# CILAB-MA/gpudrive_lab

Hardware: AMD Instinct MI355X
Metric: agent-steps/sec at 1024 worlds x 64 agents; achieved HBM GB/s on obs kernel (higher is better)
Workload: dtype f32

## Files before the change

### gpudrive_lab_amd/csrc/map_obs_rank.hip

```cpp
#include <hip/hip_runtime.h>

#include <algorithm>
#include <type_traits>

#include "engine.hpp"
#include "gd_math.hpp"
#include "rank_heap.hpp"

namespace gd {

namespace {

constexpr int K = GD_MAP_OBS_K;
constexpr int CAP = GD_RANK_CAP;
constexpr int NCP = GD_RANK_NCP;
constexpr int SPL = GD_RANK_SPL;
constexpr int KT = GD_RANK_KT;
constexpr int TILE = 32;
constexpr int CAP_LONG = GD_RANK_CAP_LONG;
template <int CAP_T>
struct RankGeo {
    static constexpr bool LONG = CAP_T > CAP;
    static constexpr int NG = CAP_T / 64;
    static constexpr int NMAX = CAP_T - 8;
    static constexpr int NB = CAP_T;
    static constexpr int NLIN = CAP_T * 3 / 5;
    static constexpr int TSH = LONG ? 6 : 5;
    static constexpr int RSH = LONG ? 4 : 5;
    static constexpr int KTN = LONG ? GD_RANK_KT_LONG : GD_RANK_KT;
};
constexpr int NB = RankGeo<CAP>::NB;
static_assert(K + (NCP - 1) * TILE >= CAP && K + (NCP - 1) * 64 >= CAP_LONG, "a checkpoint slot for every tile of candidates");
static_assert(CAP % 64 == 0 && NB % 128 == 0 && CAP < 2047 && CAP_LONG % 640 == 0 && CAP_LONG < 4095, "geometry; less + 1 fits 11 / 12 bits");
static_assert(SPL >= K + 31 && SPL <= CAP && KT >= CAP / 16 + 1, "every slot the finish looks up; an entry per 16 slots + the last");
constexpr int RK_FAR = 1 << 30;
constexpr int RK_TIES = 1 << 30;

__device__ __forceinline__ void wave_sync() {
    __builtin_amdgcn_fence(__ATOMIC_RELEASE, "wavefront");
    __builtin_amdgcn_wave_barrier();
    __builtin_amdgcn_fence(__ATOMIC_ACQUIRE, "wavefront");
}

__device__ __forceinline__ int wave_incl_scan(int v) {
    v += __builtin_amdgcn_update_dpp(0, v, 0x111, 0xf, 0xf, false);
    v += __builtin_amdgcn_update_dpp(0, v, 0x112, 0xf, 0xf, false);
    v += __builtin_amdgcn_update_dpp(0, v, 0x114, 0xf, 0xf, false);
    v += __builtin_amdgcn_update_dpp(0, v, 0x118, 0xf, 0xf, false);
    v += __builtin_amdgcn_update_dpp(0, v, 0x142, 0xa, 0xf, false);
    v += __builtin_amdgcn_update_dpp(0, v, 0x143, 0xc, 0xf, false);
    return v;
}

#define GD_DPP_SELF(v, ctrl, rows) __builtin_amdgcn_update_dpp((v), (v), (ctrl), (rows), 0xf, false)
__device__ __forceinline__ int wave_max(int v) {
    v = max(v, GD_DPP_SELF(v, 0x111, 0xf));
    v = max(v, GD_DPP_SELF(v, 0x112, 0xf));
    v = max(v, GD_DPP_SELF(v, 0x114, 0xf));
    v = max(v, GD_DPP_SELF(v, 0x118, 0xf));
    v = max(v, GD_DPP_SELF(v, 0x142, 0xa));
    v = max(v, GD_DPP_SELF(v, 0x143, 0xc));
    return __builtin_amdgcn_readlane(v, 63);
}
__device__ __forceinline__ float wave_max_nonneg(float f) { return __int_as_float(wave_max(__float_as_int(f))); }
__device__ __forceinline__ float wave_min_nonneg(float f) { return __int_as_float(~wave_max(~__float_as_int(f))); }
__device__ __forceinline__ int wave_sum(int v) { return __builtin_amdgcn_readlane(wave_incl_scan(v), 63); }

#ifndef GD_NT_SCAN_STORE
#define GD_NT_SCAN_STORE 0
#endif
#ifndef GD_NT_WORDS_LOAD
#define GD_NT_WORDS_LOAD 1
#endif
#ifndef GD_NT_FINISH_LOAD
#define GD_NT_FINISH_LOAD 1
#endif
#ifndef GD_NT_REPLAY_LOAD
#define GD_NT_REPLAY_LOAD 1
#endif
typedef unsigned int u4v __attribute__((ext_vector_type(4)));
typedef unsigned int u2v __attribute__((ext_vector_type(2)));
template <typename T>
__device__ __forceinline__ T stream_load(const T *p) { return __builtin_nontemporal_load(p); }
template <typename T>
__device__ __forceinline__ void stream_store(T v, T *p) { __builtin_nontemporal_store(v, p); }
__device__ __forceinline__ uint4 stream_load(const uint4 *p) {
    const u4v v = __builtin_nontemporal_load(reinterpret_cast<const u4v *>(p));
    return make_uint4(v.x, v.y, v.z, v.w);
}
__device__ __forceinline__ void stream_store(uint4 v, uint4 *p) {
    u4v t; t.x = v.x; t.y = v.y; t.z = v.z; t.w = v.w;
    __builtin_nontemporal_store(t, reinterpret_cast<u4v *>(p));
}
__device__ __forceinline__ uint2 stream_load(const uint2 *p) {
    const u2v v = __builtin_nontemporal_load(reinterpret_cast<const u2v *>(p));
    return make_uint2(v.x, v.y);
}
__device__ __forceinline__ void stream_store(uint2 v, uint2 *p) {
    u2v t; t.x = v.x; t.y = v.y;
    __builtin_nontemporal_store(t, reinterpret_cast<u2v *>(p));
}

__device__ __forceinline__ int audited(const DevSim &d, int idx, int size) {
    if ((unsigned int)idx < (unsigned int)size) return idx;
    atomicAdd(&d.rk_hist[GD_RANK_AUDIT], 1);
    return idx < 0 ? 0 : size - 1;
}

__device__ __forceinline__ bool rank_lt(unsigned int a, unsigned int b, unsigned int tm = 31u) { return (a | tm) < b; }

constexpr int SCAN_TILE = 2048;

template <int A_T>
__global__ __launch_bounds__(256) void k_knn_scan(DevSim d) {
    if (d.gate_any && *d.any_reset == 0) return;
    constexpr int HALVES = A_T / 64;
    const int w = blockIdx.x / HALVES, a0 = (blockIdx.x % HALVES) * 64;
    const int tid = threadIdx.x, wave = tid >> 6, lane = tid & 63;
    const int n = d.shape[w * 2 + 0];
    if (a0 >= n) return;
    const int a = a0 + lane;
    const bool live = a < n;
    const size_t i = (size_t)w * A_T + a;
    const size_t WA = (size_t)d.W * A_T;
    const int r0 = d.road_off[w];
    const int R = d.road_off[w + 1] - r0;

    __shared__ __attribute__((aligned(16))) float2 s_xy[SCAN_TILE];
    __shared__ unsigned short s_first[NCP][64];
    __shared__ float s_thr[NCP][64];
    __shared__ int s_ncp[64];
    __shared__ unsigned int s_needy[2];
    constexpr int TB = 8;
    __shared__ __attribute__((aligned(16))) unsigned int s_tr[4][TB][65];
    static_assert(sizeof(float4) * 64 + sizeof(float) * 192 <= sizeof(unsigned int) * 4 * TB * 65 && 4 * 256 * 4 <= sizeof(float2) * SCAN_TILE, "aliases fit");
    float4 *const s_hdr = reinterpret_cast<float4 *>(&s_tr[0][0][0]);
    float *const s_bx = reinterpret_cast<float *>(s_hdr + 64), *const s_by = s_bx + 64, *const s_bm = s_by + 64;
    unsigned int (*const s_hist)[256] = reinterpret_cast<unsigned int (*)[256]>(s_xy);

    float ex = 0.f, ey = 0.f;
    if (live) { ex = d.px[i]; ey = d.py[i]; }
    unsigned long long ranked = 0ull;
    int list_base = 0;
    if (wave == 0) {
        int ncp = 0;
        float4 h0 = make_float4(0.f, 0.f, __int_as_float(0), 0.f), h1 = h0;
        if (live) { h0 = d.cp_hdr[i]; h1 = d.cp_hdr[WA + i]; }
        s_hdr[lane] = h0;
        wave_sync();
        if (live) {
            const float4 bb = d.road_bbox[w];
            const float ddx = fmaxf(fmaxf(bb.x - ex, ex - bb.z), 0.f), ddy = fmaxf(fmaxf(bb.y - ey, ey - bb.w), 0.f);
            const float far = d.p.observationRadius * 1.01f + 1.f;
            int state = 1, reason = -1;
            if (R >= K && ddx * ddx + ddy * ddy > far * far) {
                state = RK_FAR;
                d.sel_hdr[i * 2] = make_float4(ex, ey, d.qw[i], d.qz[i]);
                d.sel_hdr[i * 2 + 1] = make_float4(__int_as_float(0), __int_as_float(r0), 0.f, 0.f);
                d.cp_hdr[i] = make_float4(ex, ey, __int_as_float(0), 0.f);
            } else {
                const int n0 = __float_as_int(h0.z), n1 = __float_as_int(h1.z);
                const float m0 = n0 > 0 ? sqrtf((ex - h0.x) * (ex - h0.x) + (ey - h0.y) * (ey - h0.y)) : __builtin_inff();
                const float m1 = n1 > 0 ? sqrtf((ex - h1.x) * (ex - h1.x) + (ey - h1.y) * (ey - h1.y)) : __builtin_inff();
                int set = m1 < m0 ? 1 : 0;
                float move = set ? m1 : m0;
                int n_cp = set ? n1 : n0;
                size_t src = i;
                if (move > 6.f) {
                    float best = move;
                    int donor = -1;
                    for (int j = 0; j < 64; j++) {
                        const float4 hj = s_hdr[j];
                        const float dj = __float_as_int(hj.z) > 0 ? sqrtf((ex - hj.x) * (ex - hj.x) + (ey - hj.y) * (ey - hj.y)) : __builtin_inff();
                        if (dj < best) { best = dj; donor = j; }
                    }
                    if (donor >= 0) {
                        move = best;
                        set = 0;
                        n_cp = __float_as_int(s_hdr[donor].z);
                        src = (size_t)w * A_T + a0 + donor;
                    }
                }
                const bool eligible = R >= K && R >= d.rk_min_roads && R <= d.rk_max_roads;
                const int grp = (int)(i / 32);
                const bool bypass = eligible && d.rk_streak[grp] >= 3 && ((d.rk_hist[513] + grp) & 63) != 0;
                const float iw = d.qw[i], iz = d.qz[i];
                const float z2 = iz * iz;
                const float det = (1.f - 2.f * z2) * (1.f - 2.f * z2) + 4.f * z2 * (iw * iw);
                const float margin = 1.00001f / fminf(det, 1.f);
                if (!eligible || bypass) {
                    state = 0;
                    ncp = 0;
                    reason = bypass ? -5 : -2;
                    d.rk_fallback[i / 32] = 1;
                } else if (n_cp <= 0 || move > 6.f) {
                    ncp = -1;
                    s_bx[lane] = ex; s_by[lane] = ey; s_bm[lane] = margin;
                } else {
                    ncp = n_cp;
                    const unsigned short *cr = d.cp_road + ((size_t)set * WA + src) * NCP;
                    const float *ct = d.cp_T + ((size_t)set * WA + src) * NCP;
                    float t = 1.f;
                    for (int q = 0; q < ncp; q++) {
                        t = ct[q];
                        const float reach = sqrtf(t) * 1.0001f + move * 1.0001f + 1e-3f;
                        float thr = reach * reach * 1.0001f * margin;
                        if (!(thr >= 0.f)) thr = __builtin_inff();
                        s_first[q][lane] = cr[q];
                        s_thr[q][lane] = thr;
                    }
                    d.rk_tl[i] = t;
                }
            }
            d.rk_n[i] = state;
            d.rk_ticket[i] = reason;
            if (state == RK_FAR) ncp = 0;
        }
        s_ncp[lane] = ncp;
        {
            const unsigned long long nd = __ballot(ncp < 0);
            if (lane == 0) { s_needy[0] = (unsigned int)nd; s_needy[1] = (unsigned int)(nd >> 32); }
        }
        if (ncp < 0) ncp = 1;
        ranked = __ballot(ncp > 0);
    }
    __syncthreads();
    {
        const unsigned long long needy = (unsigned long long)s_needy[0] | (unsigned long long)s_needy[1] << 32;
        if (needy != 0ull) {
            constexpr int BASE = (127 - 2) << 4;
            unsigned int *hist = s_hist[wave];
            int turn = 0;
            for (unsigned long long rest = needy; rest != 0ull; rest &= rest - 1ull, turn++) {
                if ((turn & 3) != wave) continue;
                const int al = __ffsll((long long)rest) - 1;
                const float bx = s_bx[al], by = s_by[al], mg = s_bm[al];
#pragma unroll
                for (int k = 0; k < 4; k++) hist[k * 64 + lane] = 0u;
                if (lane == 0) { s_first[0][al] = (unsigned short)((K / 32) * 32); s_thr[0][al] = __builtin_inff(); }
                const float ratio = exp2f(log2f(fmaxf((float)R / 256.f, 1.f)) / (float)(NCP - 2));
                float pf = 256.f, tlast = __builtin_inff();
                int pq = 256, q = 1;
                float2 nxt = lane < R ? d.road_xy[r0 + lane] : make_float2(0.f, 0.f);
                for (int rb = 0; rb < R; rb += 64) {
                    const float2 xy = nxt;
                    if (rb + 64 + lane < R) nxt = d.road_xy[r0 + rb + 64 + lane];
                    if (rb + lane < R) {
                        const float dx = xy.x - bx, dy = xy.y - by;
                        const float d2 = __builtin_fmaf(dx, dx, dy * dy);
                        atomicAdd(&hist[min(255, max(0, (int)(__float_as_uint(d2) >> 19) - BASE))], 1u);
                    }
                    if (rb + 64 == pq && q < NCP && pq < R) {
                        wave_sync();
                        const uint4 h = reinterpret_cast<const uint4 *>(hist)[lane];
                        const int own = (int)(h.x + h.y + h.z + h.w);
                        const int incl = wave_incl_scan(own), excl = incl - own;
                        int jb = 0, before = excl;
                        if (before + (int)h.x < K) { before += (int)h.x; jb = 1;
                            if (before + (int)h.y < K) { before += (int)h.y; jb = 2;
                                if (before + (int)h.z < K) { jb = 3; } } }
                        const unsigned long long cross = __ballot(excl < K && incl >= K);
                        const int Lc = __ffsll((long long)cross) - 1;
                        const int bucket = 4 * Lc + __builtin_amdgcn_readlane(jb, Lc);
                        const float T = bucket >= 255 ? __builtin_inff() : __uint_as_float((unsigned int)(bucket + 1 + BASE) << 19);
                        if (lane == 0) {
                            const float reach = sqrtf(T) * 1.0001f + 1e-3f;
                            float thr = reach * reach * 1.0001f * mg * 1.001f;
                            if (!(thr >= 0.f)) thr = __builtin_inff();
                            s_first[q][al] = (unsigned short)min(pq, 65535);
                            s_thr[q][al] = thr;
                        }
                        tlast = T;
                        q++;
                        pf *= ratio;
                        pq = max(pq + 64, ((int)pf + 63) & ~63);
                    }
                }
                if (lane == 0) {
                    s_ncp[al] = q;
                    d.rk_tl[(size_t)w * A_T + a0 + al] = tlast < 1e30f ? tlast : 1.f;
                }
            }
            __syncthreads();
        }
    }
    const int ncp = s_ncp[lane];
    if (__syncthreads_or(ncp > 0 ? 1 : 0) == 0) return;
    int q = -1;
    const int nch = (R + 31) >> 5;
    uint32_t *words = d.rk_words + ((size_t)w * A_T + a0) * GD_RANK_NCH;
    for (int tile = 0; tile < R; tile += SCAN_TILE) {
        __syncthreads();
        for (int r = tile + tid; r < min(R, tile + SCAN_TILE); r += 256) s_xy[r - tile] = d.road_xy[r0 + r];
        __syncthreads();
        if (wave == 0 && ranked != 0ull && lane == 0 && tile + SCAN_TILE >= R)
            list_base = atomicAdd(&d.rk_hist[528 + (blockIdx.x & 7)], __popcll(ranked));
#pragma clang loop unroll(disable)
        for (int c_first = (tile >> 5) + wave * 16; c_first < (tile >> 5) + wave * 16 + 16 && c_first < nch; c_first += TB) {
#pragma clang loop unroll(disable)
            for (int k = 0; k < TB; k++) {
                const int c = c_first + k;
                unsigned int wd = 0;
                if (c < nch) {
                    const int base = c << 5;
                    while (q + 1 < ncp && (int)s_first[q + 1][lane] <= base) q++;
                    const float thr = q >= 0 ? s_thr[q][lane] : __builtin_inff();
                    const float2 *t = s_xy + (base - tile);
#pragma unroll
                    for (int j = 31; j >= 0; j--) {
                        const float2 xy = t[j];
                        const float dx = xy.x - ex, dy = xy.y - ey;
                        const float d2 = __builtin_fmaf(dx, dx, dy * dy);
                        wd = __builtin_amdgcn_alignbit(wd, __float_as_uint(d2 - thr), 31);
                    }
                    if (base < K) wd |= K - base >= 32 ? 0xffffffffu : (1u << (K - base)) - 1u;
                    const int left = R - base;
                    if (left < 32) wd &= (1u << left) - 1u;
                }
                s_tr[wave][k][lane] = wd;
            }
            wave_sync();
#pragma unroll
            for (int it = 0; it < TB; it++) {
                const int ag = it * 8 + (lane >> 3), k = lane & 7;
#if GD_NT_SCAN_STORE
                if (c_first + k < nch && s_ncp[ag] > 0) stream_store(s_tr[wave][k][ag], words + (size_t)ag * GD_RANK_NCH + c_first + k);
#else
                if (c_first + k < nch && s_ncp[ag] > 0) words[(size_t)ag * GD_RANK_NCH + c_first + k] = s_tr[wave][k][ag];
#endif
            }
            wave_sync();
        }
    }
    if (wave == 0 && ranked != 0ull) {
        list_base = __builtin_amdgcn_readfirstlane(list_base);
        if (ncp > 0)
            d.rk_list[(size_t)(blockIdx.x & 7) * WA + audited(d, list_base + __popcll(ranked & ((1ull << lane) - 1ull)), (int)WA)] = (int)i;
    }
}

template <int CAP_T>
struct RankLds {
    union {
        unsigned short cidx[CAP_T];
        struct {
            float skey[CAP_T];
            unsigned short spos[CAP_T];
        } s;
        unsigned short spc[CAP_T];
    };
    unsigned int cnt2[RankGeo<CAP_T>::NB / 2];
};
static_assert(sizeof(RankLds<CAP>) <= 10240 && sizeof(RankLds<CAP_LONG>) <= 20480, "sixteen / eight waves per CU");

constexpr int WPL = GD_RANK_NCH / 64;
struct RankIn {
    int i, state, r0, R, li;
    float ex, ey, iw, iz, t_last;
    unsigned int wd[WPL];
};
template <typename T>
__device__ __forceinline__ T uniform_load(const T *p) {
    return *reinterpret_cast<const __attribute__((address_space(4))) T *>(reinterpret_cast<uintptr_t>(p));
}
template <int A_T>
__device__ __forceinline__ RankIn rank_fetch(const DevSim &d, const int *list, int li, int count, int lane) {
    RankIn in;
    in.li = li;
    in.i = li < count ? uniform_load(list + li) : 0;
    in.state = li < count ? uniform_load(d.rk_n + in.i) : 0;
    const int w = in.i / A_T;
    in.r0 = uniform_load(d.road_off + w);
    in.R = uniform_load(d.road_off + w + 1) - in.r0;
    in.ex = uniform_load(d.px + in.i); in.ey = uniform_load(d.py + in.i);
    in.iw = uniform_load(d.qw + in.i); in.iz = -uniform_load(d.qz + in.i);
    in.t_last = uniform_load(d.rk_tl + in.i);
    const int nch = (in.R + 31) >> 5;
    const uint32_t *words = d.rk_words + (size_t)in.i * GD_RANK_NCH;
#pragma unroll
    for (int k = 0; k < WPL; k++) {
        const int c = k * 64 + lane;
        in.wd[k] = (in.state == 1 && c < nch) ? (GD_NT_WORDS_LOAD ? stream_load(words + c) : words[c]) : 0u;
    }
    return in;
}

#ifdef GD_CLOCKS
struct PhaseClock {
    unsigned int prev, sum[8];
    __device__ __forceinline__ void mark(int n) {
        const unsigned int t = (unsigned int)__builtin_amdgcn_s_memtime();
        sum[n] += t - prev;
        prev = t;
    }
};
#define GD_PHASE(n) clk.mark(n)
#else
struct PhaseClock {};
#define GD_PHASE(n)
#endif
template <int A_T, int CAP_T>
__device__ __forceinline__ void rank_agent(const DevSim &d, const RankIn &in, int lane, RankLds<CAP_T> &L, PhaseClock &clk, int next_entry,
                                           int count, const int *list, RankIn &nxt) {
    using G = RankGeo<CAP_T>;
    constexpr int NB = G::NB, NLIN = G::NLIN, NMAX = G::NMAX;
    constexpr unsigned int TM = (1u << G::RSH) - 1u;
    if (__builtin_amdgcn_readfirstlane(in.state) != 1) {
        nxt = rank_fetch<A_T>(d, list, next_entry, count, lane);
        return;
    }
    auto uni = [](int v) -> int { return __builtin_amdgcn_readfirstlane(v); };
    auto unif = [](float v) -> float { return __int_as_float(__builtin_amdgcn_readfirstlane(__float_as_int(v))); };
    const int i = uni(in.i), r0 = uni(in.r0), R = uni(in.R);
    const int group = i / 32;
    constexpr int NG = G::NG;

    const int nch = (R + 31) >> 5;
    {
        int mine = 0;
#pragma unroll
        for (int k = 0; k < WPL; k++) {
            const int c = k * 64 + lane;
            unsigned int wd = k * 64 < nch ? in.wd[k] : 0u;
            if (k == 0) wd = c < K / 32 ? 0u : (c == K / 32 ? wd & ~((1u << (K % 32)) - 1u) : wd);
            mine += __popc(wd);
        }
        const int total = K + wave_sum(mine);
        if (total > NMAX) {
            if (lane == 0) {
                bool passed_on = false;
                if (!G::LONG && total <= RankGeo<CAP_LONG>::NMAX) {
                    const int slot = atomicAdd(&d.rk_hist[GD_RH_LONG], 1);
                    if (slot < d.rk_nlong) {
                        d.rk_longlist[slot] = i;
                        passed_on = true;
                    }
                }
                if (!passed_on) {
                    d.rk_n[i] = 0;
                    d.rk_ticket[i] = -3;
                    d.rk_fallback[group] = 1;
                }
            }
            nxt = rank_fetch<A_T>(d, list, next_entry, count, lane);
            return;
        }
    }

    static_assert(K == 200 && CAP >= 256, "roads 0..K-1: four stores per lane");
#pragma unroll
    for (int q = 0; q < 4; q++)
        if (q * 64 + lane < K) L.cidx[q * 64 + lane] = (unsigned short)(q * 64 + lane);
    int nin = K;
#pragma unroll
    for (int k = 0; k < WPL; k++) {
        if (k * 64 >= nch) break;
        const int c = k * 64 + lane;
        unsigned int wd = in.wd[k];
        if (k == 0) wd = c < K / 32 ? 0u : (c == K / 32 ? wd & ~((1u << (K % 32)) - 1u) : wd);
        const int pc = __popc(wd);
#ifdef GD_CLOCKS
        clk.sum[7] += (unsigned int)wave_max(pc) << 8;
#endif
        const int incl = wave_incl_scan(pc);
        int pos = nin + incl - pc;
        nin += __builtin_amdgcn_readlane(incl, 63);
        while (wd) {
            L.cidx[pos++] = (unsigned short)((c << 5) + __ffs(wd) - 1);
            wd &= wd - 1u;
        }
    }
    wave_sync();
    const int bin = 255 - min(255, (nin - K) / 5);
    int ticket = 0;
    if (lane == 0) ticket = bin << 20 | atomicAdd(&d.rk_hist[bin], 1);
    GD_PHASE(1);
    if (GD_DIAG_IS(d.rk_dbg, 1)) {
        nxt = rank_fetch<A_T>(d, list, next_entry, count, lane);
        return;
    }
    if (lane <= (nin - K) >> G::TSH) {
        const int road = (int)L.cidx[K - 1 + (lane << G::TSH)];
        d.cp_road[(size_t)i * NCP + lane] = (unsigned short)(lane ? min(65535, (road + 1 + 31) & ~31) : (K / 32) * 32);
    }
    constexpr int GQ = 5;
    static_assert(NG % GQ == 0, "whole groups");
    int ci[NG];
#pragma unroll
    for (int g0 = 0; g0 < NG; g0 += GQ) {
#pragma unroll
        for (int u = 0; u < GQ; u++) ci[g0 + u] = 0;
        if (g0 * 64 < nin) {
            int v[GQ];
#pragma unroll
            for (int u = 0; u < GQ; u++) v[u] = (int)L.cidx[(g0 + u) * 64 + lane];
#pragma unroll
            for (int u = 0; u < GQ; u++) ci[g0 + u] = (g0 + u) * 64 + lane < nin ? v[u] : 0;
        }
    }
    wave_sync();
    const float ex = unif(in.ex), ey = unif(in.ey), iw = unif(in.iw), iz = unif(in.iz);
    const float kmax = d.radius_key_max;
    const float2 *rxy = d.road_xy + r0;
    float key[NG];
    const float t_last = unif(in.t_last);
    float split = (t_last > 0.f && t_last < 1e30f) ? t_last * 1.5f : 1.f;
    int nle = 0, nlow = 0;
    float kmax_seen = 0.f, kmin_seen = __builtin_inff();
#pragma unroll
    for (int g0 = 0; g0 < NG; g0 += GQ) {
#pragma unroll
        for (int u = 0; u < GQ; u++) key[g0 + u] = 0.f;
        if (g0 * 64 < nin) {
            float2 xy[GQ];
#pragma unroll
            for (int u = 0; u < GQ; u++) xy[u] = rxy[(unsigned int)ci[g0 + u]];
            static_assert(GQ == 5, "operand list");
            asm volatile("" : "+v"(xy[0].x), "+v"(xy[0].y), "+v"(xy[1].x), "+v"(xy[1].y), "+v"(xy[2].x), "+v"(xy[2].y),
                              "+v"(xy[3].x), "+v"(xy[3].y), "+v"(xy[4].x), "+v"(xy[4].y));
#pragma unroll
            for (int u = 0; u < GQ; u++) {
                const int g = g0 + u;
                key[g] = ego_dist2(ex, ey, iw, iz, xy[u].x, xy[u].y);
                const bool on = g * 64 + lane < nin;
                nle += ((on & (key[g] <= kmax)) ? 1 : 0) + ((on & (key[g] < split)) ? 1 << 16 : 0);
                kmax_seen = fmaxf(kmax_seen, on ? key[g] : 0.f);
                kmin_seen = fminf(kmin_seen, on ? key[g] : __builtin_inff());
            }
        }
    }
    nxt = rank_fetch<A_T>(d, list, next_entry, count, lane);
    nle = wave_sum(nle);
    kmax_seen = wave_max_nonneg(kmax_seen);
    kmin_seen = wave_min_nonneg(kmin_seen);
    nlow = nle >> 16;
    nle &= 0xffff;
    GD_PHASE(2);
    if (GD_DIAG_IS(d.rk_dbg, 2)) return;

    for (int b = lane; b < NB / 2; b += 64) L.cnt2[b] = 0u;
    wave_sync();
    const bool jumped = nlow * 4 < nin || nlow == nin;
    const float lin_lo = jumped ? kmin_seen : 0.f;
    const int nlin = jumped ? NB : NLIN;
    const float lin_scale = jumped ? (float)NB / fmaxf(kmax_seen - kmin_seen, 1e-30f) : (float)NLIN / split;
    if (jumped) split = __builtin_inff();
    const unsigned int split_bits = __float_as_uint(split);
    const float log_scale = (float)(NB - NLIN) / (float)(max(__float_as_uint(kmax_seen), split_bits + 1u) - split_bits + 1u);
    auto bucket_of = [&](float k) -> int {
        if (k < split) return min(nlin - 1, max(0, (int)((k - lin_lo) * lin_scale)));
        return NLIN + min(NB - NLIN - 1, (int)((float)(__float_as_uint(k) - split_bits) * log_scale));
    };
#pragma unroll
    for (int g = 0; g < NG; g++) {
        if (g * 64 < nin) {
            const int b = bucket_of(key[g]);
            ci[g] |= b << 16;
            if (g * 64 + lane < nin) atomicAdd(&L.cnt2[b >> 1], 1u << ((b & 1) * 16));
        }
    }
    wave_sync();
    {
        constexpr int WPB = NB / 64 / 2;
        static_assert(WPB * 128 == NB, "whole counter words per lane");
        unsigned int own[WPB];
        int sum = 0;
#pragma unroll
        for (int k = 0; k < WPB; k++) { own[k] = L.cnt2[lane * WPB + k]; sum += (int)(own[k] & 0xffffu) + (int)(own[k] >> 16); }
        int run = wave_incl_scan(sum) - sum;
#pragma unroll
        for (int k = 0; k < WPB; k++) {
            const int lo = run, hi = run + (int)(own[k] & 0xffffu);
            run = hi + (int)(own[k] >> 16);
            L.cnt2[lane * WPB + k] = (unsigned int)lo | (unsigned int)hi << 16;
        }
    }
    wave_sync();
    GD_PHASE(3);
    if (GD_DIAG_IS(d.rk_dbg, 3)) return;
#pragma unroll
    for (int g0 = 0; g0 < NG; g0 += GQ) {
        if (g0 * 64 < nin) {
            int sl[GQ];
#pragma unroll
            for (int u = 0; u < GQ; u++) {
                const int b = ci[g0 + u] >> 16, sh = (b & 1) * 16;
                const unsigned int one = (g0 + u) * 64 + lane < nin ? 1u << sh : 0u;
                sl[u] = (int)((atomicAdd(&L.cnt2[b >> 1], one) >> sh) & 0xffffu);
            }
#pragma unroll
            for (int u = 0; u < GQ; u++) {
                if ((g0 + u) * 64 + lane < nin) {
                    L.s.skey[sl[u]] = key[g0 + u];
                    L.s.spos[sl[u]] = (unsigned short)((g0 + u) * 64 + lane);
                }
            }
        }
    }
    wave_sync();
    GD_PHASE(4);
    if (GD_DIAG_IS(d.rk_dbg, 4)) return;
    const unsigned short *cur16 = reinterpret_cast<const unsigned short *>(L.cnt2);
    unsigned int eqmask = 0u;
    float *const kt_row = G::LONG ? d.rk_kt_long + (size_t)uni(in.li) * G::KTN : d.rk_kt + (size_t)i * G::KTN;
    if (lane == 0) kt_row[(nin + 15) >> 4] = kmax_seen;
    constexpr int U = 4, M = 6, STEP = 4;
    const int lim = nin;
    if (lane < 8) L.s.skey[nin + lane] = __builtin_inff();
    wave_sync();
#pragma unroll
    for (int g0 = 0; g0 < NG; g0 += U) {
        if (g0 * 64 >= nin) break;
        int s0[U], s1[U], less[U], eq[U], longest = 0;
#pragma unroll
        for (int u = 0; u < U; u++) {
            const int b = ci[g0 + u] >> 16;
            s0[u] = b ? (int)cur16[b - 1] : 0;
            s1[u] = (g0 + u) * 64 + lane < nin ? (int)cur16[b] : s0[u];
        }
#pragma unroll
        for (int u = 0; u < U; u++) {
            float mk[M];
            static_assert(M <= 8, "end markers");
#pragma unroll
            for (int k = 0; k < M; k++) mk[k] = L.s.skey[s0[u] + k];
            less[u] = s0[u];
            eq[u] = 0;
            longest = max(longest, s1[u] - s0[u]);
#pragma unroll
            for (int k = 0; k < M; k++) {
                less[u] += mk[k] < key[g0 + u] ? 1 : 0;
                eq[u] += mk[k] == key[g0 + u] ? 1 : 0;
            }
        }
        longest = wave_max(longest);
        if (GD_DIAG_IS(d.rk_dbg, 7)) longest = 0;
#ifdef GD_DIAG
        if (lane == 0 && d.rk_dbg == 9) atomicMax(&d.rk_hist[514], longest);
#endif
        for (int j = M; j < longest; j += STEP) {
            float mkk[U][STEP];
#pragma unroll
            for (int u = 0; u < U; u++)
#pragma unroll
                for (int k = 0; k < STEP; k++) mkk[u][k] = L.s.skey[min(s0[u] + j + k, lim)];
#pragma unroll
            for (int u = 0; u < U; u++)
#pragma unroll
                for (int k = 0; k < STEP; k++) {
                    less[u] += mkk[u][k] < key[g0 + u] ? 1 : 0;
                    eq[u] += mkk[u][k] == key[g0 + u] ? 1 : 0;
                }
        }
#pragma unroll
        for (int u = 0; u < U; u++) {
            const bool on = (g0 + u) * 64 + lane < nin;
            eqmask |= ((eq[u] > 1) & on) ? 1u << (g0 + u) : 0u;
            ci[g0 + u] = (ci[g0 + u] & 0xffff) | ((less[u] + 1) << (16 + G::RSH));
            const int j = (less[u] + 15) >> 4;
            if (on && (j << 4) < less[u] + eq[u]) kt_row[j] = key[g0 + u];
        }
    }
    int too_many_ties = 0;
    const bool has_tie = __ballot(eqmask != 0u) != 0ull;
    if (has_tie) {
#pragma clang loop unroll(disable)
        for (int g = 0; g * 64 < nin; g++) {
            if (__ballot((eqmask >> g) & 1u) == 0ull) continue;
            int cg = 0;
#pragma unroll
            for (int k = 0; k < NG; k++) cg = k == g ? ci[k] : cg;
            int tie = 0;
            if ((eqmask >> g) & 1u) {
                const int less_g = (int)((unsigned int)cg >> (16 + G::RSH)) - 1, p = g * 64 + lane;
                int lo = 0, hi = NB - 1;
#pragma clang loop unroll(disable)
                while (lo < hi) {
                    const int mid = (lo + hi) >> 1;
                    if ((int)cur16[mid] > less_g) hi = mid; else lo = mid + 1;
                }
                const int b = lo;
                const int first = b ? (int)cur16[b - 1] : 0, end = (int)cur16[b];
                float kg = 0.f;
                for (int m = first; m < end; m++) kg = (int)L.s.spos[m] == p ? L.s.skey[m] : kg;
                for (int m = first; m < end; m++) tie += (L.s.skey[m] == kg ? 1 : 0) & ((int)L.s.spos[m] < p ? 1 : 0);
            }
            too_many_ties |= tie > (int)TM ? 1 : 0;
#pragma unroll
            for (int k = 0; k < NG; k++) ci[k] |= k == g ? (tie & (int)TM) << 16 : 0;
        }
    }
    wave_sync();
    GD_PHASE(5);
    if (GD_DIAG_IS(d.rk_dbg, 5)) return;
    if (__ballot(too_many_ties != 0) != 0ull) {
        if (lane == 0) {
            d.rk_n[i] = 0;
            d.rk_ticket[i] = ticket | RK_TIES;
            d.rk_fallback[group] = 1;
        }
        return;
    }
    unsigned short *const E_row = G::LONG ? d.rk_E_long + (size_t)uni(in.li) * CAP_LONG : d.rk_E + (size_t)i * CAP;
    const unsigned int ulane = (unsigned int)lane;
#pragma unroll
    for (int g = 0; g < NG; g++) {
        if (g * 64 < nin) {
            if (g * 64 + lane < nin) {
                const unsigned int e = (unsigned int)ci[g] >> 16;
                stream_store((unsigned short)e, E_row + (g * 64u + ulane));
                const int slot = (int)(e >> G::RSH) - 1 + (int)(e & TM);
                if (slot < SPL) L.spc[slot] = (unsigned short)(ci[g] & 0xffff);
            }
        }
    }
    wave_sync();
    {
        static_assert(SPL == 256, "four slots per lane");
        const uint2 v = reinterpret_cast<const uint2 *>(L.spc)[lane];
        stream_store(v, reinterpret_cast<uint2 *>(d.rk_spc + (size_t)i * SPL) + ulane);
    }
    if (lane == 0) {
        d.rk_n[i] = nin | (nle << 16) | (has_tie ? 1 << 28 : 0) | (G::LONG ? 1 << 29 : 0);
        if (G::LONG) d.rk_longslot[i] = uni(in.li);
        d.rk_ticket[i] = ticket;
    }
    GD_PHASE(6);
}

template <int A_T, int CAP_T>
__global__ __launch_bounds__(64, CAP_T > CAP ? 2 : 4) void k_knn_rank(DevSim d) {
    if (d.gate_any && *d.any_reset == 0) return;
    __shared__ RankLds<CAP_T> L;
    constexpr bool LONG = RankGeo<CAP_T>::LONG;
    const int stride = LONG ? (int)gridDim.x : (int)(gridDim.x >> 3);
    const int xcd = blockIdx.x & 7;
    const int count = LONG ? min(uniform_load(d.rk_hist + GD_RH_LONG), d.rk_nlong) : uniform_load(d.rk_hist + 528 + xcd);
    const int *list = LONG ? d.rk_longlist : d.rk_list + (size_t)xcd * d.W * A_T;
    int t = LONG ? (int)blockIdx.x : (int)(blockIdx.x >> 3);
    RankIn cur = rank_fetch<A_T>(d, list, t, count, threadIdx.x);
    PhaseClock clk;
#ifdef GD_CLOCKS
    for (int k = 0; k < 8; k++) clk.sum[k] = 0u;
    clk.prev = (unsigned int)__builtin_amdgcn_s_memtime();
#endif
    for (; t < count; t += stride) {
        RankIn nxt;
        GD_PHASE(0);
        rank_agent<A_T, CAP_T>(d, cur, threadIdx.x, L, clk, t + stride, count, list, nxt);
        wave_sync();
        cur = nxt;
    }
#ifdef GD_CLOCKS
    if (threadIdx.x == 0)
        for (int k = 0; k < 8; k++) atomicAdd(reinterpret_cast<unsigned int *>(&d.rk_hist[516 + k]), clk.sum[k] >> 8);
#endif
}

#ifndef GD_RANK_AWR
#define GD_RANK_AWR 64
#endif
constexpr int AWR = GD_RANK_AWR;
typedef unsigned int __attribute__((may_alias)) heap_u32;
typedef unsigned short __attribute__((may_alias)) heap_u16;
struct RankHeap {
    heap_u32 *pr;
    __device__ __forceinline__ unsigned int pair(int j) const { return pr[j * AWR]; }
    __device__ __forceinline__ unsigned int get(int g) const {
        return reinterpret_cast<const heap_u16 *>(pr + (g >> 1) * AWR)[g & 1];
    }
    __device__ __forceinline__ void set(int g, unsigned int v) const {
        reinterpret_cast<heap_u16 *>(pr + (g >> 1) * AWR)[g & 1] = (unsigned short)v;
    }
    __device__ __forceinline__ void set_pair(int j, unsigned int v) const { pr[j * AWR] = v; }
};
static_assert(rank_heap::NPAIR == 128, "s_pair of k_knn_replay");

__global__ __launch_bounds__(256) void k_knn_order(DevSim d) {
    if (d.gate_any && *d.any_reset == 0) return;
    __shared__ int s_part[4];
    __shared__ int s_start[256];
    const int tl = threadIdx.x;
    const int c = d.rk_hist[tl];
    const int incl = wave_incl_scan(c);
    if ((tl & 63) == 63) s_part[tl >> 6] = incl;
    __syncthreads();
    int before = 0;
    for (int k = 0; k < (tl >> 6); k++) before += s_part[k];
    s_start[tl] = before + incl - c;
    if (blockIdx.x == 0 && tl == 255) {
        d.rk_hist[512] = before + incl;
        d.rk_hist[513]++;
        for (int x = 0; x < 8; x++) d.rk_hist[528 + x] = 0;
        d.rk_hist[GD_RH_LONG] = 0;
    }
#ifdef GD_CLOCKS
    if (blockIdx.x == 0) d.rk_hist[256 + tl] = 0;
#endif
    __syncthreads();
    const int t = blockIdx.x * 256 + tl;
    if (t >= d.live_count) return;
    const int i = d.live_list[t];
    const int ticket = d.rk_ticket[i];
    if (ticket < 0) return;
    d.rk_order[audited(d, s_start[(ticket >> 20) & 255] + (ticket & 0xfffff), d.W * d.A)] = i;
}

#ifdef GD_CLOCKS
struct ReplayClock {
    unsigned int prev, first, ph[5];
    __device__ __forceinline__ void start() { first = prev = (unsigned int)__builtin_amdgcn_s_memrealtime(); }
    __device__ __forceinline__ void mark(int n) {
        const unsigned int t = (unsigned int)__builtin_amdgcn_s_memrealtime();
        ph[n] = t - prev;
        prev = t;
    }
};
#define GD_RPHASE(n) rclk.mark(n)
#else
#define GD_RPHASE(n)
#endif
__global__ __launch_bounds__(64) void k_knn_replay(DevSim d) {
    if (d.gate_any && *d.any_reset == 0) return;
    const int lane = threadIdx.x;
#ifdef GD_CLOCKS
    ReplayClock rclk;
    rclk.start();
#endif
    if (blockIdx.x == 0)
        for (int k = 0; k < 4; k++) d.rk_hist[k * 64 + lane] = 0;
    const int li = blockIdx.x * AWR + lane;
    constexpr int NPAIR = 128;
    __shared__ unsigned int s_pair[NPAIR * AWR];
    const RankHeap H{reinterpret_cast<heap_u32 *>(s_pair) + (lane % AWR)};
    int i = 0, n = 0, has_tie = 0, is_long = 0;
    if (lane < AWR && li < d.rk_hist[512]) {
        i = d.rk_order[li];
        const int packed = d.rk_n[i];
        n = packed & 0xffff;
        has_tie = (packed >> 28) & 1;
        is_long = (packed >> 29) & 1;
        if (d.rk_fallback[i / 32] != 0) n = 0;
    }
    const bool on = n >= K;
    if (__ballot(on) == 0ull) return;
    const unsigned short *E = (on && is_long) ? d.rk_E_long + (size_t)d.rk_longslot[i] * CAP_LONG : d.rk_E + (size_t)i * CAP;
    const unsigned int tm = is_long ? 15u : 31u;
    const int tsh = is_long ? 6 : 5;

    const bool wave_ties = __ballot(on && has_tie) != 0ull;
    rank_heap::TieTrack tt{rank_heap::NO_TIE};
    GD_RPHASE(0);
    {
        const uint4 *src = reinterpret_cast<const uint4 *>(E);
        unsigned int w[K / 2];
#pragma unroll
        for (int k = 0; k < K / 8; k++) {
            const uint4 v = stream_load(src + k);
            w[k * 4 + 0] = v.x;
            w[k * 4 + 1] = v.y;
            w[k * 4 + 2] = v.z;
            w[k * 4 + 3] = v.w;
        }
        if (lane < AWR) rank_heap::fill_pairs<K>(H, w);
        if (wave_ties && __ballot(on && rank_heap::any_tie(w, tm)) != 0ull) {
            tt = rank_heap::track_of(w, tm);
            if (!on) tt.tg = rank_heap::NO_TIE;
        }
    }
    const bool heap_ties = __ballot(tt.tl()) != 0ull;
    GD_RPHASE(1);
    if (on) {
        if (heap_ties) rank_heap::make_heap<K, true>(H, tm);
        else rank_heap::make_heap<K, false>(H, tm);
    }
    GD_RPHASE(2);
    unsigned int r[8];
#pragma unroll
    for (int j = 1; j < 8; j++) r[j] = H.get(j);
    unsigned int last = H.get(K);
    if (lane < AWR) H.set(K, 0u);
    unsigned short *cpe = d.rk_cpe + (size_t)i * NCP;
    if (on) cpe[0] = (unsigned short)r[1];

    int nmax = n;
#pragma unroll
    for (int off = 32; off > 0; off >>= 1) nmax = max(nmax, __shfl_xor(nmax, off));
    const uint4 *blocks = reinterpret_cast<const uint4 *>(E + K);
    uint4 cur = on ? (GD_NT_REPLAY_LOAD ? stream_load(blocks) : blocks[0]) : make_uint4(0u, 0u, 0u, 0u);
    uint4 nxt = on ? (GD_NT_REPLAY_LOAD ? stream_load(blocks + 1) : blocks[1]) : make_uint4(0u, 0u, 0u, 0u);
#ifdef GD_CLOCKS
    int n_ins = 0;
    int blk_all = 0, blk_ties = 0, blk_checked = 0;
    int n_chk = 0, n_redo = 0;
    const auto wave_any = [&](bool f) -> bool {
        const bool a = __ballot(f) != 0ull;
        n_chk++;
        n_redo += a ? 1 : 0;
        return a;
    };
#else
    const auto wave_any = [](bool f) -> bool { return __ballot(f) != 0ull; };
#endif
    auto replay = [&](auto mixed_tag) {
        constexpr bool MIXED = decltype(mixed_tag)::value;
        static_assert(TILE == 32, "four blocks of eight candidates per checkpoint");
#pragma clang loop unroll(disable)
        for (int p0 = K; p0 < nmax; p0 += TILE) {
#pragma clang loop unroll(disable)
            for (int pb = p0; pb < min(p0 + TILE, nmax); pb += 8) {
                const uint4 w8 = cur;
                cur = nxt;
                nxt = GD_NT_REPLAY_LOAD ? stream_load(blocks + ((pb - K) >> 3) + 2) : blocks[((pb - K) >> 3) + 2];
                const unsigned int wd[4] = {w8.x, w8.y, w8.z, w8.w};
                const int left = n - pb;
                int ins;
                if (MIXED && __ballot(on && rank_heap::block_has_tie(wd, left, tm)) != 0ull) {
                    ins = rank_heap::block_rounds<K, rank_heap::TIES>(H, r, last, wd, left, tm, tt);
#ifdef GD_CLOCKS
                    blk_ties++;
#endif
                } else if (MIXED && __ballot(tt.tl()) != 0ull) {
                    ins = rank_heap::block_rounds<K, rank_heap::CHECKED>(H, r, last, wd, left, tm, tt, wave_any);
#ifdef GD_CLOCKS
                    blk_checked++;
#endif
                } else {
                    ins = rank_heap::block_rounds<K, rank_heap::PLAIN>(H, r, last, wd, left, tm, tt);
                }
#ifdef GD_CLOCKS
                n_ins += ins;
                blk_all++;
#else
                (void)ins;
#endif
            }
            const int after = p0 - K + TILE;
            if (p0 + TILE - 1 < n && (after & ((1 << tsh) - 1)) == 0) cpe[after >> tsh] = (unsigned short)r[1];
        }
    };
    if (wave_ties) replay(std::true_type{});
    else replay(std::false_type{});
    GD_RPHASE(3);
#ifdef GD_CLOCKS
    {
        const int tot_ins = wave_sum(n_ins), tot_cand = wave_sum(on ? n - K : 0), longest = wave_max(on ? n - K : 0);
        if (lane == 0) {
            atomicAdd(&d.rk_hist[526], tot_ins);
            atomicAdd(&d.rk_hist[525], tot_cand);
            if (blockIdx.x == 0) atomicAdd(&d.rk_hist[524], longest);
        }
    }
#endif
    if (lane < AWR) {
        H.set(K, last);
#pragma unroll
        for (int j = 1; j < 8; j++) H.set(j, r[j]);
    }
    if (on) {
        unsigned int *out = d.rk_heap + (size_t)i * GD_RANK_HEAP_DW;
#pragma clang loop unroll(disable)
        for (int j = 0; j < GD_RANK_HEAP_DW; j += 4) {
            uint4 v;
            v.x = j + 0 <= K / 2 ? H.pair(j + 0) : 0u;
            v.y = j + 1 <= K / 2 ? H.pair(j + 1) : 0u;
            v.z = j + 2 <= K / 2 ? H.pair(j + 2) : 0u;
            v.w = j + 3 <= K / 2 ? H.pair(j + 3) : 0u;
            stream_store(v, reinterpret_cast<uint4 *>(out + j));
        }
    }
#ifdef GD_CLOCKS
    GD_RPHASE(4);
    const int w_chk = wave_sum(n_chk), w_redo = wave_sum(n_redo);
    if (lane == 0) {
        const int total = (int)(rclk.prev - rclk.first);
        if (blockIdx.x < 32) {
            int *row = d.rk_hist + 256 + blockIdx.x * 7;
            for (int k = 0; k < 5; k++) row[k] = (int)rclk.ph[k];
            row[5] = (wave_ties ? 1 : 0) | (blk_ties << 1) | (blk_checked << 10) | (blk_all << 20);
            row[6] = total;
        }
        atomicAdd(&d.rk_hist[480], wave_ties ? 1 : 0);
        atomicAdd(&d.rk_hist[481], 1);
        atomicMax(&d.rk_hist[482], total);
        atomicMax(&d.rk_hist[wave_ties ? 483 : 484], total);
        atomicAdd(&d.rk_hist[485], blk_ties);
        atomicAdd(&d.rk_hist[486], wave_ties ? blk_all : 0);
        atomicAdd(&d.rk_hist[487], blk_checked);
        atomicAdd(&d.rk_hist[488], w_chk);
        atomicAdd(&d.rk_hist[489], w_redo);
    }
#endif
}

template <int A_T>
__global__ __launch_bounds__(256) void k_knn_finish(DevSim d) {
    if (d.gate_any && *d.any_reset == 0) return;
    const int tid = threadIdx.x, wave = tid >> 6, lane = tid & 63;
    const int li = blockIdx.x * 4 + wave;
    const int ranked_agents = d.rk_hist[512];
    const int i = d.rk_order[min(li, d.W * A_T - 1)];
    constexpr int NP = (K + 63) / 64;
    const int w = i / A_T;
    const int fell_back = d.rk_fallback[i / 32];
    const int packed = d.rk_n[i];
    const int r0 = d.road_off[w], r1 = d.road_off[w + 1];
    const float ex = d.px[i], ey = d.py[i];
    const float qw = d.qw[i], qz = d.qz[i];
    const uint32_t steps_left = d.steps[i];
    const int long_slot = d.rk_longslot[i];
    const unsigned int *hp = d.rk_heap + (size_t)i * GD_RANK_HEAP_DW;
    unsigned int hpair[NP];
#pragma unroll
    for (int ps = 0; ps < NP; ps++) hpair[ps] = GD_NT_FINISH_LOAD ? stream_load(hp + min((ps * 64 + lane + 1) >> 1, GD_RANK_HEAP_DW - 1)) : hp[min((ps * 64 + lane + 1) >> 1, GD_RANK_HEAP_DW - 1)];
    static_assert(SPL == 256, "four slots per lane");
    const uint2 spc4 = GD_NT_FINISH_LOAD ? stream_load(reinterpret_cast<const uint2 *>(d.rk_spc + (size_t)i * SPL) + lane) : reinterpret_cast<const uint2 *>(d.rk_spc + (size_t)i * SPL)[lane];
    const unsigned int cp_e = d.rk_cpe[(size_t)i * NCP + min(lane, NCP - 1)];
    const unsigned short cp_r = d.cp_road[(size_t)i * NCP + min(lane, NCP - 1)];
    static_assert(NP == 4, "operand list");
    asm volatile("" ::"v"(fell_back), "v"(packed), "v"(ex), "v"(ey), "v"(qw), "v"(qz), "v"(steps_left), "v"(long_slot), "v"(hpair[0]),
                 "v"(hpair[1]), "v"(hpair[2]), "v"(hpair[3]), "v"(spc4.x), "v"(spc4.y), "v"(cp_e), "v"(cp_r), "s"(r0), "s"(r1));
    if (li >= ranked_agents || fell_back != 0) return;
    const int n = packed & 0xffff, nle = (packed >> 16) & 0xfff;
    if (packed <= 0 || packed == RK_FAR || n < K) return;
    const bool is_long = ((packed >> 29) & 1) != 0;
    const int rsh = is_long ? 4 : 5, tsh = is_long ? 6 : 5;
    const unsigned int tm = (1u << rsh) - 1u;
    const int cp_slot = (int)(cp_e >> rsh) - 1 + (int)(cp_e & tm);
    const int ncp = 1 + ((n - K) >> tsh);
    const float *kt_row = is_long ? d.rk_kt_long + (size_t)long_slot * GD_RANK_KT_LONG : d.rk_kt + (size_t)i * KT;
    float cp_t = 0.f;
    if (lane < ncp) cp_t = kt_row[min(max((cp_slot + 15) >> 4, 0), (n + 15) >> 4)];
    __shared__ unsigned short s_spc[4][SPL];
    __shared__ unsigned short s_don[4][K];
    __shared__ unsigned int s_bm[4][GD_RANK_NCH];
    __shared__ unsigned short s_wp[4][GD_RANK_NCH];
    __shared__ unsigned int s_sorted[4][K];
    unsigned short *don = s_don[wave];
    unsigned int *bm = s_bm[wave];
    const unsigned long long lower = (1ull << lane) - 1ull;
    {
        reinterpret_cast<uint2 *>(s_spc[wave])[lane] = spc4;
#pragma unroll
        for (int k = 0; k < GD_RANK_NCH / 64; k++) bm[k * 64 + lane] = 0u;
    }
    wave_sync();

    int road[NP];
    bool inr[NP];
    unsigned long long fl[NP];
    int m = 0;
#pragma unroll
    for (int ps = 0; ps < NP; ps++) {
        const int t = ps * 64 + lane, g = t + 1;
        road[ps] = 0;
        inr[ps] = false;
        if (t < K) {
            const unsigned int p2 = hpair[ps];
            const unsigned int e = (g & 1) ? p2 >> 16 : p2 & 0xffffu;
            const int less = (int)(e >> rsh) - 1;
            road[ps] = s_spc[wave][audited(d, less + (int)(e & tm), min(n, SPL))];
            inr[ps] = less < nle;
        }
        fl[ps] = __ballot(inr[ps]);
        m += __popcll(fl[ps]);
    }
    if (m < K) {
        int above = 0;
#pragma unroll
        for (int ps = NP - 1; ps >= 0; ps--) {
            const int t = ps * 64 + lane;
            if (t < K && t >= m && inr[ps]) don[above + __popcll(fl[ps] & ~lower & ~(1ull << lane))] = (unsigned short)road[ps];
            above += __popcll(fl[ps]);
        }
        wave_sync();
        int before = 0;
        int in_before = 0;
#pragma unroll
        for (int ps = 0; ps < NP; ps++) {
            const int t = ps * 64 + lane;
            if (t < m && !inr[ps]) {
                const int h = (t - before) - __popcll(fl[ps] & lower) + (before - in_before);
                road[ps] = don[h];
            }
            before += 64;
            in_before += __popcll(fl[ps]);
        }
    }
    const int R = r1 - r0;
#pragma unroll
    for (int ps = 0; ps < NP; ps++) {
        const int t = ps * 64 + lane;
        if (t < m) atomicOr(&bm[audited(d, road[ps], R) >> 5], 1u << (road[ps] & 31));
    }
    wave_sync();
    {
        constexpr int WL = GD_RANK_NCH / 64;
        unsigned int own[WL];
        int sum = 0;
#pragma unroll
// ... 70 lines not shown
```

Baseline: 64.17 million.

## Prefetch road tiles into registers and spread checkpoint loads across the block in kNN scan

Road coordinate tiles are now loaded into registers before the header phase and before each next tile is scanned, so global-load latency overlaps with compute instead of sitting between two barriers. Checkpoint threshold loads, previously done serially per lane by wave 0, are now spread across all 256 threads, and the LDS arrays are padded to stride 65 to avoid bank conflicts. The inner distance loop reads float4 from LDS with double-buffered register sets. Threshold lookahead and the keep mask are hoisted out of the loops. Optional clock instrumentation is added. The cost is higher register pressure from the prefetch arrays, which could lower occupancy.

```diff
diff --git a/gpudrive_lab_amd/csrc/map_obs_rank.hip b/gpudrive_lab_amd/csrc/map_obs_rank.hip
--- a/gpudrive_lab_amd/csrc/map_obs_rank.hip
+++ b/gpudrive_lab_amd/csrc/map_obs_rank.hip
@@ -110,6 +110,36 @@
 __device__ __forceinline__ bool rank_lt(unsigned int a, unsigned int b, unsigned int tm = 31u) { return (a | tm) < b; }
 
 constexpr int SCAN_TILE = 2048;
+constexpr int CPS = 65;
+
+#ifdef GD_CLOCKS
+struct ScanClock {
+    unsigned int prev, sum[6];
+    __device__ __forceinline__ void start() {
+        for (int k = 0; k < 6; k++) sum[k] = 0u;
+        prev = (unsigned int)__builtin_amdgcn_s_memtime();
+    }
+    __device__ __forceinline__ void mark(int n) {
+        const unsigned int t = (unsigned int)__builtin_amdgcn_s_memtime();
+        sum[n] += t - prev;
+        prev = t;
+    }
+    __device__ __forceinline__ void flush(const DevSim &d, unsigned int *lds) const {
+        __syncthreads();
+        if ((threadIdx.x & 63) == 0)
+            for (int k = 0; k < 6; k++) lds[(threadIdx.x >> 6) * 6 + k] = sum[k];
+        __syncthreads();
+        if (threadIdx.x < 6)
+            atomicAdd(reinterpret_cast<unsigned int *>(&d.rk_hist[490 + 6 * (blockIdx.x % 3) + threadIdx.x]),
+                      (lds[threadIdx.x] + lds[6 + threadIdx.x] + lds[12 + threadIdx.x] + lds[18 + threadIdx.x]) >> 2);
+    }
+};
+#define GD_SPHASE(n) sclk.mark(n)
+#define GD_SFLUSH() sclk.flush(d, &s_tr[0][0][0])
+#else
+#define GD_SPHASE(n)
+#define GD_SFLUSH()
+#endif
 
 template <int A_T>
 __global__ __launch_bounds__(256) void k_knn_scan(DevSim d) {
@@ -119,6 +149,10 @@
     const int tid = threadIdx.x, wave = tid >> 6, lane = tid & 63;
     const int n = d.shape[w * 2 + 0];
     if (a0 >= n) return;
+#ifdef GD_CLOCKS
+    ScanClock sclk;
+    sclk.start();
+#endif
     const int a = a0 + lane;
     const bool live = a < n;
     const size_t i = (size_t)w * A_T + a;
@@ -127,35 +161,52 @@
     const int R = d.road_off[w + 1] - r0;
 
     __shared__ __attribute__((aligned(16))) float2 s_xy[SCAN_TILE];
-    __shared__ unsigned short s_first[NCP][64];
-    __shared__ float s_thr[NCP][64];
+    __shared__ unsigned short s_first[NCP * CPS];
+    __shared__ float s_thr[NCP * CPS];
     __shared__ int s_ncp[64];
     __shared__ unsigned int s_needy[2];
     constexpr int TB = 8;
     __shared__ __attribute__((aligned(16))) unsigned int s_tr[4][TB][65];
-    static_assert(sizeof(float4) * 64 + sizeof(float) * 192 <= sizeof(unsigned int) * 4 * TB * 65 && 4 * 256 * 4 <= sizeof(float2) * SCAN_TILE, "aliases fit");
+    static_assert(sizeof(float4) * 64 + sizeof(float) * 320 <= sizeof(unsigned int) * 4 * TB * 65 && 4 * 256 * 4 <= sizeof(float2) * SCAN_TILE, "aliases fit");
+    static_assert((64 * NCP) % 256 == 0 && SCAN_TILE % 256 == 0, "the row move and the tile loads deal whole rounds of the 256 threads");
     float4 *const s_hdr = reinterpret_cast<float4 *>(&s_tr[0][0][0]);
     float *const s_bx = reinterpret_cast<float *>(s_hdr + 64), *const s_by = s_bx + 64, *const s_bm = s_by + 64;
+    float *const s_mv = s_bm + 64;
+    unsigned int *const s_row = reinterpret_cast<unsigned int *>(s_mv + 64);
     unsigned int (*const s_hist)[256] = reinterpret_cast<unsigned int (*)[256]>(s_xy);
 
     float ex = 0.f, ey = 0.f;
     if (live) { ex = d.px[i]; ey = d.py[i]; }
+    float4 h0 = make_float4(0.f, 0.f, __int_as_float(0), 0.f), h1 = h0;
+    float iw = 1.f, iz = 0.f;
+    int streak = 0;
+    if (wave == 0 && live) {
+        h0 = d.cp_hdr[i]; h1 = d.cp_hdr[WA + i];
+        iw = d.qw[i]; iz = d.qz[i];
+        streak = d.rk_streak[i / 32];
+    }
+    const int selections = d.rk_hist[513];
+    const float4 bb = d.road_bbox[w];
+    constexpr int TPT = SCAN_TILE / 256;
+    float2 pre[TPT];
+    const int r_last = max(R - 1, 0);
+#pragma unroll
+    for (int k = 0; k < TPT; k++) pre[k] = d.road_xy[r0 + min(tid + k * 256, r_last)];
+    asm volatile("" : "+v"(streak));
     unsigned long long ranked = 0ull;
     int list_base = 0;
     if (wave == 0) {
         int ncp = 0;
-        float4 h0 = make_float4(0.f, 0.f, __int_as_float(0), 0.f), h1 = h0;
-        if (live) { h0 = d.cp_hdr[i]; h1 = d.cp_hdr[WA + i]; }
         s_hdr[lane] = h0;
+        s_row[lane] = 0u; s_mv[lane] = 0.f; s_bm[lane] = 1.f;
         wave_sync();
         if (live) {
-            const float4 bb = d.road_bbox[w];
             const float ddx = fmaxf(fmaxf(bb.x - ex, ex - bb.z), 0.f), ddy = fmaxf(fmaxf(bb.y - ey, ey - bb.w), 0.f);
             const float far = d.p.observationRadius * 1.01f + 1.f;
             int state = 1, reason = -1;
             if (R >= K && ddx * ddx + ddy * ddy > far * far) {
                 state = RK_FAR;
-                d.sel_hdr[i * 2] = make_float4(ex, ey, d.qw[i], d.qz[i]);
+                d.sel_hdr[i * 2] = make_float4(ex, ey, iw, iz);
                 d.sel_hdr[i * 2 + 1] = make_float4(__int_as_float(0), __int_as_float(r0), 0.f, 0.f);
                 d.cp_hdr[i] = make_float4(ex, ey, __int_as_float(0), 0.f);
             } else {
@@ -183,8 +234,7 @@
                 }
                 const bool eligible = R >= K && R >= d.rk_min_roads && R <= d.rk_max_roads;
                 const int grp = (int)(i / 32);
-                const bool bypass = eligible && d.rk_streak[grp] >= 3 && ((d.rk_hist[513] + grp) & 63) != 0;
-                const float iw = d.qw[i], iz = d.qz[i];
+                const bool bypass = eligible && streak >= 3 && ((selections + grp) & 63) != 0;
                 const float z2 = iz * iz;
                 const float det = (1.f - 2.f * z2) * (1.f - 2.f * z2) + 4.f * z2 * (iw * iw);
                 const float margin = 1.00001f / fminf(det, 1.f);
@@ -198,18 +248,8 @@
                     s_bx[lane] = ex; s_by[lane] = ey; s_bm[lane] = margin;
                 } else {
                     ncp = n_cp;
-                    const unsigned short *cr = d.cp_road + ((size_t)set * WA + src) * NCP;
-                    const float *ct = d.cp_T + ((size_t)set * WA + src) * NCP;
-                    float t = 1.f;
-                    for (int q = 0; q < ncp; q++) {
-                        t = ct[q];
-                        const float reach = sqrtf(t) * 1.0001f + move * 1.0001f + 1e-3f;
-                        float thr = reach * reach * 1.0001f * margin;
-                        if (!(thr >= 0.f)) thr = __builtin_inff();
-                        s_first[q][lane] = cr[q];
-                        s_thr[q][lane] = thr;
-                    }
-                    d.rk_tl[i] = t;
+                    s_row[lane] = (unsigned int)((size_t)set * WA + src);
+                    s_mv[lane] = move; s_bm[lane] = margin;
                 }
             }
             d.rk_n[i] = state;
@@ -225,8 +265,37 @@
         ranked = __ballot(ncp > 0);
     }
     __syncthreads();
+    const unsigned long long needy = (unsigned long long)s_needy[0] | (unsigned long long)s_needy[1] << 32;
     {
-        const unsigned long long needy = (unsigned long long)s_needy[0] | (unsigned long long)s_needy[1] << 32;
+        constexpr int PER = 64 * NCP / 256;
+        float ct[PER];
+        unsigned short cr[PER];
+#pragma unroll
+        for (int k = 0; k < PER; k++) {
+            const int e = tid + k * 256, ag = e / NCP, q = e - ag * NCP;
+            ct[k] = 1.f; cr[k] = 0;
+            if (q < s_ncp[ag] && (needy >> ag & 1ull) == 0ull) {
+                const size_t at = (size_t)s_row[ag] * NCP + q;
+                ct[k] = d.cp_T[at]; cr[k] = d.cp_road[at];
+            }
+        }
+#pragma unroll
+        for (int k = 0; k < PER; k++) {
+            const int e = tid + k * 256, ag = e / NCP, q = e - ag * NCP;
+            const int nq = s_ncp[ag];
+            if (q < nq && (needy >> ag & 1ull) == 0ull) {
+                const float t = ct[k];
+                const float reach = sqrtf(t) * 1.0001f + s_mv[ag] * 1.0001f + 1e-3f;
+                float thr = reach * reach * 1.0001f * s_bm[ag];
+                if (!(thr >= 0.f)) thr = __builtin_inff();
+                s_first[q * CPS + ag] = cr[k];
+                s_thr[q * CPS + ag] = thr;
+                if (q == nq - 1) d.rk_tl[(size_t)w * A_T + a0 + ag] = t;
+            }
+        }
+    }
+    GD_SPHASE(0);
+    {
         if (needy != 0ull) {
             constexpr int BASE = (127 - 2) << 4;
             unsigned int *hist = s_hist[wave];
@@ -237,7 +306,7 @@
                 const float bx = s_bx[al], by = s_by[al], mg = s_bm[al];
 #pragma unroll
                 for (int k = 0; k < 4; k++) hist[k * 64 + lane] = 0u;
-                if (lane == 0) { s_first[0][al] = (unsigned short)((K / 32) * 32); s_thr[0][al] = __builtin_inff(); }
+                if (lane == 0) { s_first[al] = (unsigned short)((K / 32) * 32); s_thr[al] = __builtin_inff(); }
                 const float ratio = exp2f(log2f(fmaxf((float)R / 256.f, 1.f)) / (float)(NCP - 2));
                 float pf = 256.f, tlast = __builtin_inff();
                 int pq = 256, q = 1;
@@ -267,8 +336,8 @@
                             const float reach = sqrtf(T) * 1.0001f + 1e-3f;
                             float thr = reach * reach * 1.0001f * mg * 1.001f;
                             if (!(thr >= 0.f)) thr = __builtin_inff();
-                            s_first[q][al] = (unsigned short)min(pq, 65535);
-                            s_thr[q][al] = thr;
+                            s_first[q * CPS + al] = (unsigned short)min(pq, 65535);
+                            s_thr[q * CPS + al] = thr;
                         }
                         tlast = T;
                         q++;
@@ -284,59 +353,112 @@
             __syncthreads();
         }
     }
+    GD_SPHASE(1);
+#pragma unroll
+    for (int k = 0; k < TPT; k++) s_xy[tid + k * 256] = pre[k];
     const int ncp = s_ncp[lane];
-    if (__syncthreads_or(ncp > 0 ? 1 : 0) == 0) return;
+    if (__syncthreads_or(ncp > 0 ? 1 : 0) == 0) { GD_SFLUSH(); return; }
     int q = -1;
+    float thr = __builtin_inff(), thn = thr;
+    int nb = 0x7fffffff;
+    if (ncp > 0) { nb = (int)s_first[lane]; thn = s_thr[lane]; }
+    unsigned int keep = 0u;
+#pragma unroll
+    for (int it = 0; it < 8; it++) keep |= (s_ncp[it * 8 + (lane >> 3)] > 0 ? 1u : 0u) << it;
     const int nch = (R + 31) >> 5;
     uint32_t *words = d.rk_words + ((size_t)w * A_T + a0) * GD_RANK_NCH;
+#define GD_SCAN_ROAD(X, Y)                                                                            \
+    {                                                                                                 \
+        const float dx = (X) - ex, dy = (Y) - ey;                                                     \
+        const float d2 = __builtin_fmaf(dx, dx, dy * dy);                                             \
+        wd = __builtin_amdgcn_alignbit(wd, __float_as_uint(d2 - thr), 31);  \
+    }
+#define GD_SCAN_EIGHT(V)                                                                              \
+    _Pragma("unroll") for (int j = 3; j >= 0; j--) {                                                  \
+        GD_SCAN_ROAD(V[j].z, V[j].w)                                                                  \
+        GD_SCAN_ROAD(V[j].x, V[j].y)                                                                  \
+    }                                                                                                 \
+    __builtin_amdgcn_sched_barrier(0);
+#define GD_SCAN_READ(V, P, G)                                                                         \
+    _Pragma("unroll") for (int j = 0; j < 4; j++) V[j] = (P)[(G) * 4 + j];                            \
+    __builtin_amdgcn_sched_barrier(0);
+    const float4 *const s_xy4 = reinterpret_cast<const float4 *>(s_xy);
     for (int tile = 0; tile < R; tile += SCAN_TILE) {
-        __syncthreads();
-        for (int r = tile + tid; r < min(R, tile + SCAN_TILE); r += 256) s_xy[r - tile] = d.road_xy[r0 + r];
-        __syncthreads();
-        if (wave == 0 && ranked != 0ull && lane == 0 && tile + SCAN_TILE >= R)
+        const bool more = tile + SCAN_TILE < R;
+        if (more) {
+#pragma unroll
+            for (int k = 0; k < TPT; k++) pre[k] = d.road_xy[r0 + min(tile + SCAN_TILE + tid + k * 256, r_last)];
+        }
+        if (wave == 0 && ranked != 0ull && lane == 0 && !more)
             list_base = atomicAdd(&d.rk_hist[528 + (blockIdx.x & 7)], __popcll(ranked));
+        GD_SPHASE(2);
+        const int c_lo = (tile >> 5) + wave * 16, c_hi = min(c_lo + 16, nch);
+        float4 va[4], vb[4];
+        if (c_lo < c_hi) { GD_SCAN_READ(va, s_xy4 + ((c_lo << 5) - tile) / 2, 3) }
 #pragma clang loop unroll(disable)
-        for (int c_first = (tile >> 5) + wave * 16; c_first < (tile >> 5) + wave * 16 + 16 && c_first < nch; c_first += TB) {
+        for (int c_first = c_lo; c_first < c_hi; c_first += TB) {
 #pragma clang loop unroll(disable)
             for (int k = 0; k < TB; k++) {
                 const int c = c_first + k;
                 unsigned int wd = 0;
-                if (c < nch) {
+                if (c < c_hi) {
                     const int base = c << 5;
-                    while (q + 1 < ncp && (int)s_first[q + 1][lane] <= base) q++;
-                    const float thr = q >= 0 ? s_thr[q][lane] : __builtin_inff();
-                    const float2 *t = s_xy + (base - tile);
-#pragma unroll
-                    for (int j = 31; j >= 0; j--) {
-                        const float2 xy = t[j];
-                        const float dx = xy.x - ex, dy = xy.y - ey;
-                        const float d2 = __builtin_fmaf(dx, dx, dy * dy);
-                        wd = __builtin_amdgcn_alignbit(wd, __float_as_uint(d2 - thr), 31);
+                    while (nb <= base) {
+                        q++;
+                        thr = thn;
+                        nb = 0x7fffffff;
+                        if (q + 1 < ncp) { nb = (int)s_first[(q + 1) * CPS + lane]; thn = s_thr[(q + 1) * CPS + lane]; }
                     }
+                    const float4 *t = s_xy4 + (base - tile) / 2;
+                    const float4 *tn = c + 1 < c_hi ? t + 16 : t;
+                    GD_SCAN_READ(vb, t, 2)
+                    GD_SCAN_EIGHT(va)
+                    GD_SCAN_READ(va, t, 1)
+                    GD_SCAN_EIGHT(vb)
+                    GD_SCAN_READ(vb, t, 0)
+                    GD_SCAN_EIGHT(va)
+                    GD_SCAN_READ(va, tn, 3)
+                    GD_SCAN_EIGHT(vb)
                     if (base < K) wd |= K - base >= 32 ? 0xffffffffu : (1u << (K - base)) - 1u;
                     const int left = R - base;
                     if (left < 32) wd &= (1u << left) - 1u;
                 }
                 s_tr[wave][k][lane] = wd;
             }
+            GD_SPHASE(3);
             wave_sync();
+            unsigned int out[TB];
+#pragma unroll
+            for (int it = 0; it < TB; it++) out[it] = s_tr[wave][lane & 7][it * 8 + (lane >> 3)];
 #pragma unroll
             for (int it = 0; it < TB; it++) {
                 const int ag = it * 8 + (lane >> 3), k = lane & 7;
 #if GD_NT_SCAN_STORE
-                if (c_first + k < nch && s_ncp[ag] > 0) stream_store(s_tr[wave][k][ag], words + (size_t)ag * GD_RANK_NCH + c_first + k);
+                if (c_first + k < nch && (keep >> it & 1u)) stream_store(out[it], words + (size_t)ag * GD_RANK_NCH + c_first + k);
 #else
-                if (c_first + k < nch && s_ncp[ag] > 0) words[(size_t)ag * GD_RANK_NCH + c_first + k] = s_tr[wave][k][ag];
+                if (c_first + k < nch && (keep >> it & 1u)) words[(size_t)ag * GD_RANK_NCH + c_first + k] = out[it];
 #endif
             }
             wave_sync();
-        }
-    }
+            GD_SPHASE(4);
+        }
+        if (more) {
+            __syncthreads();
+#pragma unroll
+            for (int k = 0; k < TPT; k++) s_xy[tid + k * 256] = pre[k];
+            __syncthreads();
+        }
+    }
+#undef GD_SCAN_READ
+#undef GD_SCAN_EIGHT
+#undef GD_SCAN_ROAD
     if (wave == 0 && ranked != 0ull) {
         list_base = __builtin_amdgcn_readfirstlane(list_base);
         if (ncp > 0)
             d.rk_list[(size_t)(blockIdx.x & 7) * WA + audited(d, list_base + __popcll(ranked & ((1ull << lane) - 1ull)), (int)WA)] = (int)i;
     }
+    GD_SPHASE(5);
+    GD_SFLUSH();
 }
 
 template <int CAP_T>
@@ -795,7 +917,7 @@
         d.rk_hist[GD_RH_LONG] = 0;
     }
 #ifdef GD_CLOCKS
-    if (blockIdx.x == 0) d.rk_hist[256 + tl] = 0;
+    if (blockIdx.x == 0 && tl < 234) d.rk_hist[256 + tl] = 0;
 #endif
     __syncthreads();
     const int t = blockIdx.x * 256 + tl;
```

Result: no change. 64.13 million (median of 2 runs) (-0.1%).
